# facebookresearch/dietgpu

Measured on AMD Instinct MI355X. Metric: rans_encode_decode_GBps, higher is better.
Workload: dtype u8 (byte-wise rANS on the split exponent plane of 16-bit words); 1 GPU; 256x524288 bfloat16 N(0,1), float codec, probBits 10 (BASELINE config 3); per_gpu_batch_bytes=268435456, api=C ABI: dgpu_float_compress + dgpu_float_decompress

## Files before the change

dietgpu_amd/csrc/kernels_decode.h:

```cpp
#pragma once
#include <type_traits>

#include "format.h"
#include "plan_constants.h"
#include "kernels_stats.h"

namespace dgpu {

__device__ __forceinline__ const uint8_t* locateAns(const uint8_t* archive, uint32_t ft, uint32_t* floatSize) {
  if (!ft) return archive;
  const FloatHeader fh = *(const FloatHeader*)archive;
  if (floatSize) *floatSize = fh.size;
  return archive + 16u + floatUncompDataSize(ft, fh.size);
}

struct DecodeArgs {
  BatchView in;
  BatchView out;
  uint32_t floatType;
  uint8_t* outSuccess;
  uint32_t* outSize;
  const uint32_t* inBytes;
  uint32_t numInBatch;
  uint32_t maxTiles;
// ... 128 lines not shown
  __device__ __forceinline__ void init(uint8_t* outBase, const uint8_t* archive, uint32_t, size_t first, uint32_t hl) {
    out = (uint16_t*)outBase + first + hl;
    nc = archive + 16u + first + hl;
  }
  typedef uint32_t Pre;
  typedef uint2 GroupPre;
  __device__ __forceinline__ uint32_t prefetch(uint32_t row) const { return nc[row * 32u]; }
  static __device__ __forceinline__ uint32_t joinWord(uint32_t e0, uint32_t r) {
    const uint32_t lo = joinBytes(e0, r);
    return __builtin_amdgcn_alignbit(r, lo, 1);
  }
  __device__ __forceinline__ void store(uint32_t row, uint32_t e0, uint32_t r) const {
    const uint32_t v = joinWord(e0, r);
    streamStore<kNtDecStores>(&out[row * 32u], (uint16_t)(v >> 16));
  }
  static constexpr uint32_t kXposeBytes = 512;
  __device__ __forceinline__ uint2 prefetchGroup(uint32_t g, uint32_t hl) const { return decLoad8(nc - hl + g * 256u + hl * 8u); }
  __device__ __forceinline__ void stageRow(uint32_t xpose, uint32_t j, uint32_t hl, uint32_t e0) const {
    *(LdsU16w*)(uintptr_t)(xpose + (j * 32u + hl) * 2u) = (uint16_t)(e0 >> 16);
  }
  static __device__ __forceinline__ uint32_t rotrHalves(uint32_t x) {
    typedef uint16_t u16x2w __attribute__((ext_vector_type(2)));
    const u16x2w h = __builtin_bit_cast(u16x2w, x);
    const uint32_t shifted = __builtin_bit_cast(uint32_t, (u16x2w)(h >> 1));
    uint32_t r;
    asm("v_pk_mad_u16 %0, %1, %2, %3" : "=v"(r) : "v"(x), "s"(0x80008000u), "v"(shifted));
    return r;
  }
  static __device__ __forceinline__ u32x4w joinGroup(uint32_t xpose, uint32_t hl, uint2 ncb) {
    const u32x4w v = *(const LdsU4w*)(uintptr_t)(xpose + hl * 16u);
    u32x4w o;
    o.x = rotrHalves(__builtin_amdgcn_perm(v.x, ncb.x, 0x07010500u));
    o.y = rotrHalves(__builtin_amdgcn_perm(v.y, ncb.x, 0x07030502u));
    o.z = rotrHalves(__builtin_amdgcn_perm(v.z, ncb.y, 0x07010500u));
    o.w = rotrHalves(__builtin_amdgcn_perm(v.w, ncb.y, 0x07030502u));
    return o;
  }
  __device__ __forceinline__ void flushGroup(uint32_t xpose, uint32_t g, uint32_t hl, uint2 ncb) const {
    const u32x4w o = joinGroup(xpose, hl, ncb);
    u32x4w* dst = (u32x4w*)(out - hl + g * 256u + hl * 8u);
    if (kNtDecStores) __builtin_nontemporal_store(o, dst);
    else *dst = o;
  }
};

template <>
struct RowSink<kFloat32> {
  uint32_t* out;
  const uint16_t* nc2;
  const uint8_t* nc1;
  __device__ __forceinline__ void init(uint8_t* outBase, const uint8_t* archive, uint32_t floatSize, size_t first, uint32_t hl) {
    out = (uint32_t*)outBase + first + hl;
    nc2 = (const uint16_t*)(archive + 16u) + first + hl;
    nc1 = archive + 16u + 2u * (size_t)roundUp(floatSize, 8u) + first + hl;
  }
  typedef uint32_t Pre;
  typedef uint2 GroupPre;
  __device__ __forceinline__ uint32_t prefetch(uint32_t row) const {
    return ((uint32_t)nc1[row * 32u] << 16) | nc2[row * 32u];
  }
  __device__ __forceinline__ void store(uint32_t row, uint32_t e0, uint32_t r) const {
    const uint32_t v = (e0 & 0xff000000u) | r;
    streamStore<kNtDecStores>(&out[row * 32u], (uint32_t)__builtin_amdgcn_alignbit(v, v, 1));
  }
  static __device__ __forceinline__ uint32_t joinWord(uint32_t e0, uint32_t r) {
    const uint32_t v = (e0 & 0xff000000u) | r;
    return (uint32_t)__builtin_amdgcn_alignbit(v, v, 1);
  }
  static constexpr uint32_t kXposeBytes = 0;
  __device__ __forceinline__ uint2 prefetchGroup(uint32_t, uint32_t) const { return make_uint2(0, 0); }
  __device__ __forceinline__ void stageRow(uint32_t, uint32_t, uint32_t, uint32_t) const {}
  __device__ __forceinline__ void flushGroup(uint32_t, uint32_t, uint32_t, uint2) const {}
};

template <uint32_t FT>
__device__ __forceinline__ float accWiden16(uint32_t h);
template <>
__device__ __forceinline__ float accWiden16<kFloat16>(uint32_t h) { return (float)__builtin_bit_cast(_Float16, (uint16_t)h); }
template <>
__device__ __forceinline__ float accWiden16<kBFloat16>(uint32_t h) { return __builtin_bit_cast(float, h << 16); }
__device__ __forceinline__ uint32_t accAdd(uint32_t acc, float v) { return __builtin_bit_cast(uint32_t, __fadd_rn(__builtin_bit_cast(float, acc), v)); }
typedef u32x4w u32x4w4 __attribute__((aligned(4)));

struct AccumPre {
  uint32_t r, acc;
  __device__ __forceinline__ AccumPre() = default;
  __device__ __forceinline__ AccumPre(uint32_t) : r(0), acc(0) {}
};
struct AccumGroupPre {
  uint2 nc;
  u32x4w a0, a1;
};

constexpr uint32_t kStatsSlotsLarge = 16, kStatsSlotsSmall = 8;
__host__ __device__ constexpr uint32_t decStatsSlots(uint32_t tileBlocks) { return tileBlocks <= 4u ? kStatsSlotsSmall : kStatsSlotsLarge; }
__host__ __device__ constexpr uint32_t decStatsBinBytes(uint32_t tileBlocks) { return kNumSymbols * decStatsSlots(tileBlocks) * 4u; }
typedef __attribute__((address_space(3))) uint32_t LdsU32w;
template <bool kStats>
struct AccumBins {};
template <>
struct AccumBins<true> {
  uint32_t bins;
};

template <bool kInRegisters>
struct AccumScale {};
template <>
struct AccumScale<true> {
  float scale;
  uint32_t scaleLast;
};
typedef __attribute__((address_space(3))) float LdsF32w;
__device__ __forceinline__ uint32_t accScale(uint32_t o, float f) { return __builtin_bit_cast(uint32_t, __fmul_rn(__builtin_bit_cast(float, o), f)); }

template <uint32_t FT, uint32_t kSlots = 0, bool kScaledSink = false>
struct AccumSink : AccumBins<kSlots != 0u>, AccumScale<kScaledSink && kSlots == 0u> {
  static_assert(FT == kFloat16 || FT == kBFloat16, "");
  static constexpr bool kStats = kSlots != 0u;
  static constexpr bool kScaled = kScaledSink;
  static constexpr uint32_t kStatSlots = kSlots;
  __device__ __forceinline__ bool scales() const {
    if constexpr (kStats) return this->bins != 0u;
    else return this->scaleLast != 0u;
  }
  __device__ __forceinline__ float factor() const {
    if constexpr (kStats) return *(LdsF32w*)(uintptr_t)(this->bins + kNumSymbols * kSlots * 4u);
    else return this->scale;
  }
  float* out;
  const uint8_t* nc;
  uint32_t accumulate;
  __device__ __forceinline__ void count(uint32_t o) const {
    if constexpr (kStats) {
      const uint32_t c = (castRound<FT>(o) >> (FT == kFloat16 ? 8u : 7u)) & 0xffu;
      __hip_atomic_fetch_add((LdsU32w*)(uintptr_t)(this->bins + c * (kSlots * 4u)), 1u, __ATOMIC_RELAXED, __HIP_MEMORY_SCOPE_WORKGROUP);
    }
  }
  __device__ __forceinline__ void init(uint8_t* outBase, const uint8_t* archive, uint32_t, size_t first, uint32_t hl) {
    out = (float*)outBase + first + hl;
    nc = archive + 16u + first + hl;
  }
  typedef AccumPre Pre;
  typedef AccumGroupPre GroupPre;
  __device__ __forceinline__ AccumPre prefetchAcc(uint32_t row) const {
    AccumPre p(0);
    if (accumulate) p.acc = *(const uint32_t*)&out[row * 32u];
    return p;
  }
  __device__ __forceinline__ AccumPre prefetch(uint32_t row) const {
    AccumPre p(0);
    p.r = nc[row * 32u];
    if (accumulate) p.acc = *(const uint32_t*)&out[row * 32u];
    return p;
  }
  __device__ __forceinline__ void storeWord(uint32_t row, uint32_t h, const AccumPre& p) const {
    const float v = accWiden16<FT>(h);
    uint32_t o = accumulate ? accAdd(p.acc, v) : __builtin_bit_cast(uint32_t, v);
    if constexpr (kScaled) {
      if (scales()) o = accScale(o, factor());
    }
    streamStore<kNtDecStores>((uint32_t*)&out[row * 32u], o);
    if constexpr (kStats) {
      if (this->bins) count(o);
    }
  }
  __device__ __forceinline__ void store(uint32_t row, uint32_t e0, const AccumPre& p) const {
    storeWord(row, RowSink<FT>::joinWord(e0, p.r) >> 16, p);
  }
  static constexpr uint32_t kXposeBytes = 512;
  __device__ __forceinline__ void prefetchGroupAcc(uint32_t g, uint32_t hl, AccumGroupPre& p) const {
    p.a0 = p.a1 = u32x4w{0u, 0u, 0u, 0u};
    if (accumulate) {
      const u32x4w4* src = (const u32x4w4*)(out - hl + g * 256u + hl * 8u);
      p.a0 = src[0];
      p.a1 = src[1];
    }
  }
  __device__ __forceinline__ AccumGroupPre prefetchGroup(uint32_t g, uint32_t hl) const {
    AccumGroupPre p;
    p.nc = decLoad8(nc - hl + g * 256u + hl * 8u);
    prefetchGroupAcc(g, hl, p);
    return p;
  }
  __device__ __forceinline__ void stageRow(uint32_t xpose, uint32_t j, uint32_t hl, uint32_t e0) const {
    *(LdsU16w*)(uintptr_t)(xpose + (j * 32u + hl) * 2u) = (uint16_t)(e0 >> 16);
  }
  __device__ __forceinline__ void flushGroup(uint32_t xpose, uint32_t g, uint32_t hl, const AccumGroupPre& p) const {
    flushFrom<false>(xpose, g, hl, p, u32x4w{0u, 0u, 0u, 0u});
  }
  __device__ __forceinline__ void flushWords(uint32_t g, uint32_t hl, const u32x4w& given, const AccumGroupPre& p) const {
    flushFrom<true>(0u, g, hl, p, given);
  }
  template <bool kGiven>
  __device__ __forceinline__ void flushFrom(uint32_t xpose, uint32_t g, uint32_t hl, const AccumGroupPre& p, const u32x4w& given) const {
    u32x4w w;
    if constexpr (kGiven) w = given;
    else w = RowSink<FT>::joinGroup(xpose, hl, p.nc);
    float v[8];
#pragma unroll
    for (uint32_t k = 0; k < 4u; ++k) {
      v[2u * k] = accWiden16<FT>(w[k] & 0xffffu);
      v[2u * k + 1u] = accWiden16<FT>(w[k] >> 16);
    }
    u32x4w o0, o1;
#pragma unroll
    for (uint32_t k = 0; k < 4u; ++k) {
      o0[k] = accumulate ? accAdd(p.a0[k], v[k]) : __builtin_bit_cast(uint32_t, v[k]);
      o1[k] = accumulate ? accAdd(p.a1[k], v[4u + k]) : __builtin_bit_cast(uint32_t, v[4u + k]);
    }
    if constexpr (kScaled) {
      if (scales()) {
        const float f = factor();
#pragma unroll
        for (uint32_t k = 0; k < 4u; ++k) {
          o0[k] = accScale(o0[k], f);
          o1[k] = accScale(o1[k], f);
        }
      }
    }
    u32x4w4* dst = (u32x4w4*)(out - hl + g * 256u + hl * 8u);
    if (kNtDecStores) {
      __builtin_nontemporal_store(o0, &dst[0]);
      __builtin_nontemporal_store(o1, &dst[1]);
    } else {
      dst[0] = o0;
      dst[1] = o1;
    }
    if constexpr (kStats) {
      if (this->bins) {
#pragma unroll
        for (uint32_t k = 0; k < 4u; ++k) {
          count(o0[k]);
          count(o1[k]);
        }
      }
    }
  }
};

template <uint32_t kSlots, bool kScaledSink>
struct AccumSink<kFloat32, kSlots, kScaledSink> : AccumScale<kScaledSink> {
  static_assert(kSlots == 0u, "counting sinks: the 16-bit archive types only");
  static constexpr bool kStats = false;
  static constexpr bool kScaled = kScaledSink;
  float* out;
  const uint16_t* nc2;
  const uint8_t* nc1;
  uint32_t accumulate;
  __device__ __forceinline__ void init(uint8_t* outBase, const uint8_t* archive, uint32_t floatSize, size_t first, uint32_t hl) {
    out = (float*)outBase + first + hl;
    nc2 = (const uint16_t*)(archive + 16u) + first + hl;
    nc1 = archive + 16u + 2u * (size_t)roundUp(floatSize, 8u) + first + hl;
  }
  typedef AccumPre Pre;
  typedef uint2 GroupPre;
  __device__ __forceinline__ AccumPre prefetch(uint32_t row) const {
    AccumPre p(0);
    p.r = ((uint32_t)nc1[row * 32u] << 16) | nc2[row * 32u];
    if (accumulate) p.acc = *(const uint32_t*)&out[row * 32u];
    return p;
  }
  __device__ __forceinline__ AccumPre prefetchAcc(uint32_t row) const {
    AccumPre p(0);
    if (accumulate) p.acc = *(const uint32_t*)&out[row * 32u];
    return p;
  }
  __device__ __forceinline__ void storeWord(uint32_t row, uint32_t w, const AccumPre& p) const {
    uint32_t o = accumulate ? accAdd(p.acc, __builtin_bit_cast(float, w)) : w;
    if constexpr (kScaled) {
      if (this->scaleLast != 0u) o = accScale(o, this->scale);
    }
    streamStore<kNtDecStores>((uint32_t*)&out[row * 32u], o);
  }
  __device__ __forceinline__ void store(uint32_t row, uint32_t e0, const AccumPre& p) const {
    storeWord(row, RowSink<kFloat32>::joinWord(e0, p.r), p);
  }
  static constexpr uint32_t kXposeBytes = 0;
  __device__ __forceinline__ uint2 prefetchGroup(uint32_t, uint32_t) const { return make_uint2(0, 0); }
  __device__ __forceinline__ void stageRow(uint32_t, uint32_t, uint32_t, uint32_t) const {}
  __device__ __forceinline__ void flushGroup(uint32_t, uint32_t, uint32_t, uint2) const {}
};

typedef __attribute__((address_space(3))) uint16_t LdsU16;
typedef uint32_t u32x4 __attribute__((ext_vector_type(4)));
typedef __attribute__((address_space(3))) u32x4 LdsU4;
constexpr uint32_t kRingChunkWords = 256;
constexpr uint32_t kRingBytes = 2048;
constexpr uint32_t kGroupRows = 8;

__host__ __device__ constexpr uint32_t decThreads(uint32_t tileBlocks) { return tileBlocks * 32u < 64u ? 64u : tileBlocks * 32u; }
__host__ __device__ constexpr uint32_t decXposeBytes(int P, uint32_t ft, uint32_t tileBlocks) {
  (void)P;
  if (ft == 0 && tileBlocks >= 16u) return 0u;
  return ft == kFloat32 ? 0u : 512u;
}
__host__ __device__ constexpr bool decCompactLut(int P, uint32_t tileBlocks) { return tileBlocks <= 4u || P >= 11; }
__host__ __device__ constexpr uint32_t decLutBytes(int P, uint32_t tileBlocks) {
  return decCompactLut(P, tileBlocks) ? (4u << P) : (8u << P);
}
__host__ __device__ constexpr uint32_t decLdsBytes(int P, uint32_t ft, uint32_t tileBlocks) {
  return decLutBytes(P, tileBlocks) + tileBlocks * kRingBytes + tileBlocks * decXposeBytes(P, ft, tileBlocks);
}

template <typename GroupPre>
struct DecodePreOf {
  uint4 words[4];
  GroupPre nc[2];
};
typedef DecodePreOf<uint2> DecodePre;
template <uint32_t FT, typename Sink>
__device__ __forceinline__ void decodePrefetch(DecodePreOf<typename Sink::GroupPre>& pre, const uint8_t* __restrict__ gwords, uint32_t numWords,
                                               const Sink& sink, uint32_t hl, bool wide) {
  const uint32_t paddedBytes = roundUp(numWords, kBlockAlignWords) * 2u;
#pragma unroll
  for (uint32_t k = 0; k < 4u; ++k) {
    const uint32_t off = (k * 32u + hl) * 16u;
    pre.words[k] = make_uint4(0, 0, 0, 0);
    if (off < paddedBytes) pre.words[k] = decLoad16(gwords + off);
  }
  pre.nc[0] = pre.nc[1] = typename Sink::GroupPre();
  if (wide) {
    pre.nc[0] = sink.prefetchGroup(kRowsPerBlock / 8u - 1u, hl);
    pre.nc[1] = sink.prefetchGroup(kRowsPerBlock / 8u - 2u, hl);
  }
}

template <int P, uint32_t FT, bool kFull, bool kWide = false, bool kIdleUpper = false, bool kCompact = false, bool kNoRing = false,
          bool kPre = false, bool kTail = false, typename Sink = RowSink<FT>>
__device__ __forceinline__ void decodeBlock(
    uint32_t xpose,
    uint32_t state,
    uint32_t n,
    uint32_t groups,
    const uint8_t* __restrict__ gwords,
    uint32_t numWords,
    uint32_t ringBase,
    const void* __restrict__ lutRaw,
    const Sink& sink,
    uint32_t hl,
    bool upper,
    const DecodePreOf<typename Sink::GroupPre>* pre = nullptr,
    uint32_t topRows = 0) {
  static_assert(!kPre || (kNoRing && kFull), "");
  static_assert(!kTail || (kFull && !kPre), "");
  constexpr uint32_t kMask = (1u << P) - 1u;
  const uint32_t laneMaskLt = (1u << hl) - 1u;
  auto lutAt = [&](uint32_t x) -> uint2 {
    if (kCompact) {
      const uint32_t e = ((const uint32_t*)lutRaw)[x];
      return make_uint2((e & 0xff000fffu), (e >> 12) & 0xfffu);
    }
    return ((const uint2*)lutRaw)[x];
  };
  const uint32_t paddedBytes = roundUp(numWords, kBlockAlignWords) * 2u;

  uint32_t posw = numWords;

  static_assert(!kNoRing || kFull, "whole-block staging is a full-block path");
  int lowChunk = numWords ? (int)((numWords - 1u) / kRingChunkWords) + 1 : 0;
  if (kNoRing) {
    uint4 v[4];
#pragma unroll
    for (uint32_t k = 0; k < 4u; ++k) {
      const uint32_t off = (k * 32u + hl) * 16u;
      if (kPre) {
        v[k] = pre->words[k];
      } else {
        v[k] = make_uint4(0, 0, 0, 0);
        if (off < paddedBytes) v[k] = decLoad16(gwords + off);
      }
    }
#pragma unroll
    for (uint32_t k = 0; k < 4u; ++k) {
      const uint32_t off = (k * 32u + hl) * 16u;
      if (off < paddedBytes) *(LdsU4*)(uintptr_t)(ringBase + off) = u32x4{v[k].x, v[k].y, v[k].z, v[k].w};
    }
    lowChunk = 0;
  } else {
    const int stop = numWords > 512u ? (int)((numWords - 512u) / kRingChunkWords) : 0;
    while (lowChunk > stop) {
      --lowChunk;
      const uint32_t off = (uint32_t)lowChunk * 512u + hl * 16u;
      uint4 v = make_uint4(0, 0, 0, 0);
      if (off < paddedBytes) v = decLoad16(gwords + off);
      *(LdsU4*)(uintptr_t)(ringBase | (((uint32_t)lowChunk & 3u) * 512u + hl * 16u)) = u32x4{v.x, v.y, v.z, v.w};
    }
  }
  uint4 pending = make_uint4(0, 0, 0, 0);
  int pendingChunk = -1;

  auto step = [&](bool valid) -> uint32_t {
    const uint2 e = lutAt(state & kMask);
    if (valid) state = __umul24(e.x, state >> P) + e.y;
    const bool read = valid && (state < kMinState);
    const uint64_t vote = __ballot(read);
    const uint32_t vh = upper ? (uint32_t)(vote >> 32) : (uint32_t)vote;
    posw -= __popc(vh);
    if (read) {
      const uint32_t idx = posw + __popc(vh & laneMaskLt);
      const uint32_t w = *(const LdsU16*)(uintptr_t)(((idx << 1) & (kRingBytes - 1u)) | ringBase);
      state = (state << kEncodedBits) | w;
    }
    return e.x;
  };

  typedef typename Sink::Pre Pre;
  typedef typename Sink::GroupPre GroupPre;
  uint32_t sLo = 0, sHi = 0;
  int upperSel = (upper && !kIdleUpper) ? 1 : 0;
  asm volatile("" : "+v"(upperSel));
  auto stepFull = [&]() -> uint32_t {
    const uint2 e = lutAt(state & kMask);
    state = __umul24(e.x, state >> P) + e.y;
    const bool read = state < kMinState;
    const uint64_t vote = __ballot(read);
    const uint32_t vLo = (uint32_t)vote, vHi = (uint32_t)(vote >> 32);
    const uint32_t sLoOld = sLo;
    sLo -= (uint32_t)__popc(vLo);
    sHi -= (uint32_t)__popc(vHi);
    uint32_t t = __builtin_amdgcn_mbcnt_hi(vHi, __builtin_amdgcn_mbcnt_lo(vLo, 0u));
    t = (uint32_t)(__mul24(upperSel, (int)(sHi - sLoOld)) + (int)t);
    asm volatile("" : "+v"(t));
    const uint32_t addr = kNoRing ? ((t + sLo) << 1) : ((((t + sLo) << 1) & (kRingBytes - 1u)) | ringBase);
    const uint32_t w = *(const LdsU16*)(uintptr_t)addr;
    state = read ? ((state << kEncodedBits) | w) : state;
    return e.x;
  };

  auto runGroups = [&](auto fullTag, const int gHi, const int gLo) {
    constexpr bool F = decltype(fullTag)::value;
    constexpr bool kJoinAtFlush = F && kWide;
    Pre preCur[kGroupRows], preNext[kGroupRows];
    GroupPre ncCur = GroupPre(), ncNext = GroupPre(), ncNext2 = GroupPre();
    if (kJoinAtFlush) {
      if (kPre) {
        ncCur = pre->nc[0];
        ncNext = pre->nc[1];
      } else {
        ncCur = sink.prefetchGroup((uint32_t)gHi, hl);
        ncNext = sink.prefetchGroup(gHi > gLo ? (uint32_t)(gHi - 1) : (uint32_t)gLo, hl);
      }
    }
#pragma unroll
    for (int j = 0; j < (int)kGroupRows; ++j) {
      const uint32_t row = (uint32_t)gHi * kGroupRows + j;
      preCur[j] = kJoinAtFlush ? (Pre)0 : ((F || row * 32u + hl < n) ? sink.prefetch(row) : (Pre)0);
    }

#pragma unroll 1
    for (int g = gHi; g >= gLo; --g) {
      const uint32_t gNext = g > gLo ? (uint32_t)(g - 1) : (uint32_t)gLo;
      if (kJoinAtFlush) {
        ncNext2 = sink.prefetchGroup(g > gLo + 1 ? (uint32_t)(g - 2) : (uint32_t)gLo, hl);
      } else {
#pragma unroll
        for (int j = 0; j < (int)kGroupRows; ++j) {
          const uint32_t row = gNext * kGroupRows + j;
          preNext[j] = (F || row * 32u + hl < n) ? sink.prefetch(row) : (Pre)0;
        }
      }
      if (F && !kNoRing) posw = upper ? sHi : sLo;
      if (!kNoRing) {
        if (pendingChunk >= 0) {
          *(LdsU4*)(uintptr_t)(ringBase | (((uint32_t)pendingChunk & 3u) * 512u + hl * 16u)) = u32x4{pending.x, pending.y, pending.z, pending.w};
          pendingChunk = -1;
        }
        if (lowChunk > 0 && (uint32_t)lowChunk * kRingChunkWords + 512u > posw) {
          --lowChunk;
          const uint32_t off = (uint32_t)lowChunk * 512u + hl * 16u;
          pending = (off < paddedBytes) ? decLoad16(gwords + off) : make_uint4(0, 0, 0, 0);
          pendingChunk = lowChunk;
        }
      }
#pragma unroll
      for (int j = (int)kGroupRows - 1; j >= 0; --j) {
        const uint32_t row = (uint32_t)g * kGroupRows + j;
        if (F) {
          const uint32_t e0 = stepFull();
          if (kWide) {
            if (!kIdleUpper || !upper) sink.stageRow(xpose, (uint32_t)j, hl, e0);
          } else if (!kIdleUpper || !upper) {
            sink.store(row, e0, preCur[j]);
          }
        } else {
          const bool valid = row * 32u + hl < n;
          const uint32_t e0 = step(valid);
          if (valid) sink.store(row, e0, preCur[j]);
        }
      }
      if (kJoinAtFlush) {
        if (!kIdleUpper || !upper) sink.flushGroup(xpose, (uint32_t)g, hl, ncCur);
        ncCur = ncNext;
        ncNext = ncNext2;
      } else {
#pragma unroll
        for (int j = 0; j < (int)kGroupRows; ++j) preCur[j] = preNext[j];
      }
    }
  };

  if (kTail) {
    if (topRows != 0u) runGroups(std::false_type{}, (int)(groups + divUp(topRows, kGroupRows)) - 1, (int)groups);
    if (groups == 0u) return;
  }
  if (kFull) {
    sLo = __builtin_amdgcn_readlane(posw, 0);
    sHi = __builtin_amdgcn_readlane(posw, 32);
    if (kNoRing) {
      sLo += __builtin_amdgcn_readlane(ringBase, 0) >> 1;
      sHi += __builtin_amdgcn_readlane(ringBase, 32) >> 1;
    }
  }
  runGroups(std::integral_constant<bool, kFull>{}, (int)groups - 1, 0);
}

enum class DecodeForm { kWhole, kRanged, kAccum, kReduce, kReduceStats, kReduceMixed, kReduceMixedStats, kReduceScaled, kReduceScaledStats };
template <int P, uint32_t FT, uint32_t kTileBlocks, DecodeForm kForm>
__device__ __forceinline__ void decodeTile(const DecodeArgs& a) {
  constexpr bool kRanged = kForm == DecodeForm::kRanged, kAccum = kForm == DecodeForm::kAccum;
  static_assert(kForm == DecodeForm::kWhole || kForm == DecodeForm::kRanged || kForm == DecodeForm::kAccum, "decode-reduce has a body of its own: decodeReduceTile");
  static_assert(!kAccum || FT != 0u, "accumulating decode: float archives only");
  using Sink = std::conditional_t<kAccum, AccumSink<FT ? FT : kFloat32>, RowSink<FT>>;
  constexpr uint32_t kDecThreads = decThreads(kTileBlocks);
  static_assert(kTileBlocks * kRingBytes >= 2048u, "");
  extern __shared__ __attribute__((aligned(16))) uint8_t smem[];
  uint2* sLut = (uint2*)(smem + kTileBlocks * kRingBytes);
  constexpr uint32_t kXpose = decXposeBytes(P, FT, kTileBlocks);

  const uint32_t tid = threadIdx.x;
  const uint32_t lane = tid & 63u;
  const uint32_t wave = tid >> 6;
  const bool upper = lane >= 32u;
  const uint32_t hl = lane & 31u;
  const uint32_t hw = wave * 2u + (upper ? 1u : 0u);
  uint32_t b, tile;
  if (!decodeTileOf(a, blockIdx.x, &b, &tile)) return;
  uint32_t rFirst = 0;
  uint64_t rEnd = 0;
  if constexpr (kRanged) {
    if (blockIdx.x == 0) {
      for (uint32_t e = tid; e < a.numInBatch; e += kDecThreads) {
        if (a.numBlocks[e] == 0u) {
          if (a.outSuccess) a.outSuccess[e] = 1;
          if (a.outSize) a.outSize[e] = 0;
        }
      }
    }
    if (b >= a.numInBatch) return;
    rFirst = a.firstBlock[b];
    rEnd = (uint64_t)rFirst + a.numBlocks[b];
  }
  auto rangeWords = [&](uint32_t total) -> uint32_t {
    const uint64_t lo = (uint64_t)rFirst * kBlockSize, hi = rEnd * kBlockSize;
    return lo > total ? 0u : (uint32_t)((hi < total ? hi : (uint64_t)total) - lo);
  };

  const uint8_t* archive = a.in.ptr(b);
  uint32_t floatSize = 0;
  const uint64_t inBytes = decodeInBytes(a, b);
  if (inBytes < (FT ? sizeof(FloatHeader) : sizeof(AnsHeader))) {
    if (tile == 0 && tid == 0) {
      if (a.outSuccess) a.outSuccess[b] = 0;
      if (a.outSize) a.outSize[b] = 0;
    }
    return;
  }
  if (FT) {
    const FloatHeader fh = *(const FloatHeader*)archive;
    const bool fhOk = fh.magicAndVersion == ((kFloatMagic << 16) | kFloatVersion) && (fh.options & 0xfu) == FT &&
        (kRanged || fh.size <= a.out.size(b)) &&
        (uint64_t)sizeof(FloatHeader) + floatUncompDataSize(FT, fh.size) + sizeof(AnsHeader) <= inBytes;
    if (!fhOk) {
      if (tile == 0 && tid == 0) {
        if (a.outSuccess) a.outSuccess[b] = 0;
        if (a.outSize) a.outSize[b] = kRanged ? rangeWords(fh.size) : fh.size;
      }
      return;
    }
  }
  const uint8_t* ans = locateAns(archive, FT, &floatSize);
  uint32_t block = tile * kTileBlocks + hw;
  bool inRange = true;
  if constexpr (kRanged) {
    const uint64_t blk = (uint64_t)rFirst + block;
    inRange = blk < rEnd;
    block = inRange ? (uint32_t)blk : 0u;
  }
  const bool extentKnown = inBytes != ~0ull;
  const uint32_t ansOff = ansOffsetInArchive(FT, floatSize);
  const uint32_t nbSpec = FT ? divUp(floatSize, kBlockSize) : 0u;
  const bool pdfEarly = extentKnown ? (uint64_t)ansOff + ansOverhead(0u) <= inBytes : FT != 0u;
  const bool blockEarly = FT != 0u && inRange && block < nbSpec && (!extentKnown || (uint64_t)ansOff + ansOverhead(nbSpec) <= inBytes);
  const AnsHeader header = *(const AnsHeader*)ans;
  uint2 pdfRaw = make_uint2(0u, 0u);
  if (wave == 0) pdfRaw = *(const uint2*)(pdfEarly ? ans + sizeof(AnsHeader) + 8u * lane : ans);
  uint2 bwMine = *(const uint2*)(blockEarly ? ans + ansBlockWordsOffset(nbSpec) + 8u * block : ans);
  uint32_t state = *(const uint32_t*)(blockEarly ? ans + ansStatesOffset() + 4u * (block * 32u + hl) : ans);
  const uint32_t nb = header.numBlocks;
  const uint32_t total = header.totalUncompressedWords;
  const uint32_t totalWords = header.totalCompressedWords;

  bool success = a.out.size(b) >= total;
  if constexpr (kRanged) success = (uint64_t)rFirst * kBlockSize <= total && rangeWords(total) <= a.out.size(b);
  success = success && header.magicAndVersion == ((kAnsMagic << 16) | kAnsVersion) &&
      (header.options & 0xfu) == (uint32_t)P;
  if (FT) success = success && floatSize == total;
  success = success && nb == divUp(total, kBlockSize);
  success = success && (uint64_t)ansOffsetInArchive(FT, total) + ansOverhead(nb) + 2ull * totalWords <= inBytes;
  if (!success) {
    if (tile == 0 && tid == 0) {
      if (a.outSuccess) a.outSuccess[b] = 0;
      if (a.outSize) a.outSize[b] = kRanged ? rangeWords(total) : total;
    }
    return;
  }
  uint32_t endBlock = nb, tileFirst = tile * kTileBlocks;
  if constexpr (kRanged) {
    endBlock = rEnd < nb ? (uint32_t)rEnd : nb;
    tileFirst += rFirst;
  }
  if (tileFirst >= endBlock && tile != 0) return;

  const uint2* blockWords = (const uint2*)(ans + ansBlockWordsOffset(nb));
  auto blockOk = [&](uint32_t i, uint2 bw) -> bool {
    const uint32_t want = (i + 1u < nb) ? kBlockSize : total - i * kBlockSize;
    const uint32_t words = bw.x & 0xffffu;
    return (bw.x >> 16) == want && (bw.y & (kBlockAlignWords - 1u)) == 0u &&
        (uint64_t)bw.y + roundUp(words, kBlockAlignWords) <= (uint64_t)totalWords;
  };
  bool allBlocksOk = true;
  if constexpr (kAccum) {
    for (uint32_t i = tid; i < endBlock; i += kDecThreads) allBlocksOk = blockOk(i, blockWords[i]) & allBlocksOk;
  } else if (tile == 0) {
    for (uint32_t i = rFirst + tid; i < endBlock; i += kDecThreads) allBlocksOk = allBlocksOk && blockOk(i, blockWords[i]);
  }

  bool haveBlock = inRange && block < endBlock;
  if (!haveBlock) {
    bwMine = make_uint2(0u, 0u);
    state = 0;
  } else if (!blockEarly) {
    bwMine = blockWords[block];
    state = ((const uint32_t*)(ans + ansStatesOffset()))[block * 32u + hl];
  }
  if (wave == 0 && !pdfEarly) pdfRaw = ((const uint2*)(ans + sizeof(AnsHeader)))[lane];
  uint32_t n = 0, numWords = 0, start = 0;
  if (haveBlock) {
    if (blockOk(block, bwMine)) {
      n = bwMine.x >> 16;
      numWords = bwMine.x & 0xffffu;
      start = bwMine.y;
    } else {
      haveBlock = false;
      state = 0;
    }
  }
  const uint8_t* gwords = ans + ansOverhead(nb) + 2u * (size_t)start;
  Sink sink;
  if constexpr (kAccum) sink.accumulate = a.accumulate;
  uint32_t sinkBlock = haveBlock ? block : (block & ~1u);
  if constexpr (kRanged) sinkBlock = haveBlock ? block : tileFirst + (hw & ~1u);
  sink.init(a.out.ptr(b), archive, floatSize, (size_t)sinkBlock * kBlockSize, hl);
  if constexpr (kRanged) sink.out -= (size_t)rFirst * kBlockSize;
  const uint32_t ldsBase = (uint32_t)(uintptr_t)(__attribute__((address_space(3))) uint8_t*)smem;
  const uint32_t nFirst = __shfl(n, 0, 64);
  const uint32_t nSecond = __shfl(n, 32, 64);
  const uint32_t wFirst = __shfl(numWords, 0, 64);
  const uint32_t wSecond = __shfl(numWords, 32, 64);
  const bool noRing = wFirst <= kRingBytes / 2u && wSecond <= kRingBytes / 2u;
  const bool wide = decXposeBytes(P, FT, kTileBlocks) != 0 && (kAccum || (((uintptr_t)a.out.ptr(b)) & (decOutWordBytes(FT) - 1u)) == 0);
  const bool fullPair = nFirst == kBlockSize && nSecond == kBlockSize;
  const bool fullSingle = nFirst == kBlockSize && nSecond == 0u;
  DecodePreOf<typename Sink::GroupPre> pre;
  if ((fullPair || fullSingle) && noRing) decodePrefetch<FT>(pre, gwords, numWords, sink, hl, wide);

  uint32_t* sCdf = (uint32_t*)smem;
  uint32_t* sPdf = sCdf + kNumSymbols;
  uint32_t* sPdfSum = sPdf + kNumSymbols;
  uint32_t* sWaveBad = sPdfSum + 1;
  constexpr bool kScanLut = kTileBlocks <= kDecBlocksPerSmallTile;
  uint32_t* sWaveTop = sWaveBad + 8;
  constexpr bool kCompact = decCompactLut(P, kTileBlocks);
  constexpr uint32_t kLutBytes = decLutBytes(P, kTileBlocks);
  uint8_t* sMark = (uint8_t*)sLut + kLutBytes - (1u << P);
  {
    {
      const bool waveBad = __ballot(!allBlocksOk) != 0ull;
      if (lane == 0u) sWaveBad[wave] = waveBad ? 1u : 0u;
    }
    if (kScanLut) {
      for (uint32_t i = tid; i < (1u << P) / 4u; i += kDecThreads) ((uint32_t*)sMark)[i] = 0u;
    }
    if (wave == 0) {
      const uint2 raw = pdfRaw;
      const uint32_t p0 = raw.x & 0xffffu, p1 = raw.x >> 16, p2 = raw.y & 0xffffu, p3 = raw.y >> 16;
      const uint32_t mine = p0 + p1 + p2 + p3;
      const uint32_t incl = waveInclusiveScan(mine, lane);
      const uint32_t base = incl - mine;
      ((uint4*)sCdf)[lane] = make_uint4(base, base + p0, base + p0 + p1, base + p0 + p1 + p2);
      ((uint4*)sPdf)[lane] = make_uint4(p0, p1, p2, p3);
      if (lane == 63u) *sPdfSum = incl;
    }
    __syncthreads();
    uint32_t anyBad = 0;
#pragma unroll
    for (uint32_t w = 0; w < kDecThreads / 64u; ++w) anyBad |= sWaveBad[w];
    const bool blocksOk = anyBad == 0u;
    const bool pdfOk = nb == 0u || *sPdfSum == (1u << P);
    if (tile == 0 && tid == 0) {
      if (a.outSuccess) a.outSuccess[b] = (blocksOk && pdfOk) ? 1 : 0;
      if (a.outSize) a.outSize[b] = kRanged ? rangeWords(total) : total;
    }
    if (!pdfOk || tileFirst >= endBlock) return;
    if constexpr (kAccum) {
      if (!blocksOk) return;
    }
    if constexpr (kScanLut) {
      for (uint32_t sidx = tid; sidx < kNumSymbols; sidx += kDecThreads) {
        if (sPdf[sidx]) sMark[sCdf[sidx]] = (uint8_t)sidx;
      }
      __syncthreads();
      static_assert(kCompact, "the scan build writes compact entries");
      constexpr uint32_t kWaves = kDecThreads / 64u;
      constexpr uint32_t kPart = (1u << P) / kWaves;
      static_assert(kPart % 256u == 0u, "");
      constexpr uint32_t kSteps = kPart / 256u;
      auto dmax = [](uint32_t v, uint32_t o) { return v > o ? v : o; };
      auto waveMaxScan = [&](uint32_t v) -> uint32_t {
        v = dmax(v, (uint32_t)__builtin_amdgcn_update_dpp(0, (int)v, 0x111, 0xf, 0xf, true));
        v = dmax(v, (uint32_t)__builtin_amdgcn_update_dpp(0, (int)v, 0x112, 0xf, 0xf, true));
        v = dmax(v, (uint32_t)__builtin_amdgcn_update_dpp(0, (int)v, 0x114, 0xf, 0xf, true));
        v = dmax(v, (uint32_t)__builtin_amdgcn_update_dpp(0, (int)v, 0x118, 0xf, 0xf, true));
        v = dmax(v, (uint32_t)__builtin_amdgcn_update_dpp(0, (int)v, 0x142, 0xa, 0xf, true));
        v = dmax(v, (uint32_t)__builtin_amdgcn_update_dpp(0, (int)v, 0x143, 0xc, 0xf, true));
        return v;
      };
      uint32_t m4[kSteps];
      uint32_t top = 0;
#pragma unroll
      for (uint32_t t = 0; t < kSteps; ++t) {
        m4[t] = ((const uint32_t*)sMark)[(wave * kPart + t * 256u) / 4u + lane];
        const uint32_t a01 = dmax(m4[t] & 0xffu, (m4[t] >> 8) & 0xffu);
        const uint32_t a23 = dmax((m4[t] >> 16) & 0xffu, m4[t] >> 24);
        top = dmax(top, dmax(a01, a23));
      }
      top = waveMaxScan(top);
      if (lane == 63u) sWaveTop[wave] = top;
      __syncthreads();
      uint32_t carry = 0;
      for (uint32_t w = 0; w < wave; ++w) carry = dmax(carry, sWaveTop[w]);
#pragma unroll
      for (uint32_t t = 0; t < kSteps; ++t) {
        uint32_t run[4];
        run[0] = m4[t] & 0xffu;
        run[1] = dmax(run[0], (m4[t] >> 8) & 0xffu);
        run[2] = dmax(run[1], (m4[t] >> 16) & 0xffu);
        run[3] = dmax(run[2], m4[t] >> 24);
        const uint32_t incl = waveMaxScan(run[3]);
        uint32_t excl = (uint32_t)__builtin_amdgcn_update_dpp(0, (int)incl, 0x138, 0xf, 0xf, true);
        excl = dmax(excl, carry);
        uint32_t e[4];
#pragma unroll
        for (uint32_t j = 0; j < 4u; ++j) {
          const uint32_t x = wave * kPart + t * 256u + lane * 4u + j;
          const uint32_t sym = dmax(run[j], excl);
          e[j] = (sPdf[sym] & 0xfffu) | (((x - sCdf[sym]) & 0xfffu) << 12) | (sym << 24);
        }
        ((uint4*)sLut)[(wave * kPart + t * 256u) / 4u + lane] = make_uint4(e[0], e[1], e[2], e[3]);
        carry = dmax(carry, (uint32_t)__builtin_amdgcn_readlane((int)incl, 63));
      }
    } else
    for (uint32_t x = tid; x < (1u << P); x += kDecThreads) {
      uint32_t lo = 0, hi = kNumSymbols;
#pragma unroll
      for (int it = 0; it < 8; ++it) {
        const uint32_t mid = (lo + hi) >> 1;
        const bool le = sCdf[mid] <= x;
        lo = le ? mid : lo;
        hi = le ? hi : mid;
      }
      if (kCompact) ((uint32_t*)sLut)[x] = (sPdf[lo] & 0xfffu) | (((x - sCdf[lo]) & 0xfffu) << 12) | (lo << 24);
      else sLut[x] = make_uint2((sPdf[lo] & 0xfffu) | (lo << 24), (x - sCdf[lo]) & 0xfffu);
    }
  }

  __syncthreads();

  constexpr uint32_t kLutBytesHere = decLutBytes(P, kTileBlocks);
  const uint32_t xpose = ldsBase + kTileBlocks * kRingBytes + kLutBytesHere + hw * kXpose;
  const uint32_t ringLds = ldsBase + hw * kRingBytes;
#define DGPU_DECODE_FULL(WIDE, IDLE, NORING) \
  decodeBlock<P, FT, true, WIDE, IDLE, kCompact, NORING, NORING>(xpose, state, n, kRowsPerBlock / kGroupRows, gwords, numWords, ringLds, sLut, sink, hl, upper, &pre)
  if (fullPair) {
    if (wide) {
      if (noRing) DGPU_DECODE_FULL(true, false, true); else DGPU_DECODE_FULL(true, false, false);
    } else {
      if (noRing) DGPU_DECODE_FULL(false, false, true); else DGPU_DECODE_FULL(false, false, false);
    }
  } else if (fullSingle) {
    if (wide) {
      if (noRing) DGPU_DECODE_FULL(true, true, true); else DGPU_DECODE_FULL(true, true, false);
    } else {
      if (noRing) DGPU_DECODE_FULL(false, true, true); else DGPU_DECODE_FULL(false, true, false);
    }
#undef DGPU_DECODE_FULL
  } else {
    const uint32_t maxN = nFirst > nSecond ? nFirst : nSecond;
    const uint32_t maxRows = divUp(maxN, 32u);
    const uint32_t fullRows = (nSecond ? nSecond : nFirst) / 32u;
    const uint32_t groups = fullRows / kGroupRows;
    const uint32_t topRows = maxRows - groups * kGroupRows;
    const bool tailPair = nFirst == kBlockSize && nSecond != 0u, tailSingle = nFirst != 0u && nSecond == 0u;
    if ((tailPair || tailSingle) && groups != 0u) {
#define DGPU_DECODE_TAIL(WIDE, IDLE, NORING) \
  decodeBlock<P, FT, true, WIDE, IDLE, kCompact, NORING, false, true>(xpose, state, n, groups, gwords, numWords, ringLds, sLut, sink, hl, upper, nullptr, topRows)
      if (tailPair) {
        if (wide) {
          if (noRing) DGPU_DECODE_TAIL(true, false, true); else DGPU_DECODE_TAIL(true, false, false);
        } else {
          if (noRing) DGPU_DECODE_TAIL(false, false, true); else DGPU_DECODE_TAIL(false, false, false);
        }
      } else {
        if (wide) {
          if (noRing) DGPU_DECODE_TAIL(true, true, true); else DGPU_DECODE_TAIL(true, true, false);
        } else {
          if (noRing) DGPU_DECODE_TAIL(false, true, true); else DGPU_DECODE_TAIL(false, true, false);
        }
      }
#undef DGPU_DECODE_TAIL
    } else {
      decodeBlock<P, FT, false, false, false, kCompact>(xpose, state, n, divUp(maxRows, kGroupRows), gwords, numWords, ringLds, sLut, sink, hl, upper);
    }
  }
}

constexpr uintptr_t kReduceRawTag = 1u;
__device__ __forceinline__ bool reduceIsRaw(const uint8_t* source) { return ((uintptr_t)source & kReduceRawTag) != 0u; }
typedef uint16_t u16n __attribute__((aligned(2)));
__device__ __forceinline__ uint32_t rawLoad16(const uint8_t* p) {
  return kNtEncLoads ? (uint32_t)__builtin_nontemporal_load((const u16n*)p) : (uint32_t)*(const u16n*)p;
}
__device__ __forceinline__ uint32_t rawLoad32(const uint8_t* p) {
  return kNtEncLoads ? __builtin_nontemporal_load((const uint32_t*)p) : *(const uint32_t*)p;
}
__device__ __forceinline__ u32x4w rawLoadGroup(const uint8_t* p, uint32_t align) {
  u32x4w w;
  if (align >= 16u) {
    w = kNtEncLoads ? __builtin_nontemporal_load((const u32x4w*)p) : *(const u32x4w*)p;
  } else if (align >= 4u) {
#pragma unroll
    for (uint32_t k = 0; k < 4u; ++k) w[k] = rawLoad32(p + 4u * k);
  } else {
#pragma unroll
    for (uint32_t k = 0; k < 4u; ++k) w[k] = rawLoad16(p + 4u * k) | (rawLoad16(p + 4u * k + 2u) << 16);
  }
  return w;
}
template <uint32_t FT, typename Sink>
__device__ __forceinline__ void reduceRawBlock(const Sink& sink, const uint8_t* src, uint32_t n, uint32_t hl, uint32_t align) {
  if constexpr (FT == kFloat32) {
    const uint32_t rows = n / 32u;
    uint32_t row = 0;
    for (; row + 8u <= rows; row += 8u) {
      typename Sink::Pre p[8];
      uint32_t w[8];
#pragma unroll
      for (uint32_t j = 0; j < 8u; ++j) {
        p[j] = sink.prefetchAcc(row + j);
        w[j] = rawLoad32(src + ((size_t)(row + j) * 32u + hl) * 4u);
      }
#pragma unroll
      for (uint32_t j = 0; j < 8u; ++j) sink.storeWord(row + j, w[j], p[j]);
    }
    for (; row * 32u + hl < n; ++row) {
      const typename Sink::Pre p = sink.prefetchAcc(row);
      sink.storeWord(row, rawLoad32(src + ((size_t)row * 32u + hl) * 4u), p);
    }
  } else {
    const uint32_t groups = n / (kGroupRows * 32u);
    uint32_t g = 0;
    for (; g + 4u <= groups; g += 4u) {
      typename Sink::GroupPre p[4];
      u32x4w w[4];
#pragma unroll
      for (uint32_t j = 0; j < 4u; ++j) {
        sink.prefetchGroupAcc(g + j, hl, p[j]);
        w[j] = rawLoadGroup(src + (g + j) * 512u + hl * 16u, align);
      }
#pragma unroll
      for (uint32_t j = 0; j < 4u; ++j) sink.flushWords(g + j, hl, w[j], p[j]);
    }
    for (; g < groups; ++g) {
      typename Sink::GroupPre p;
      sink.prefetchGroupAcc(g, hl, p);
      sink.flushWords(g, hl, rawLoadGroup(src + g * 512u + hl * 16u, align), p);
    }
    for (uint32_t row = groups * kGroupRows; row * 32u + hl < n; ++row) {
      const typename Sink::Pre p = sink.prefetchAcc(row);
      sink.storeWord(row, rawLoad16(src + (row * 32u + hl) * 2u), p);
    }
  }
}

__device__ __forceinline__ void reduceHandOver() {
  __builtin_amdgcn_fence(__ATOMIC_RELEASE, "workgroup");
  asm volatile("s_waitcnt vmcnt(0)" ::: "memory");
  __builtin_amdgcn_s_barrier();
  __builtin_amdgcn_fence(__ATOMIC_ACQUIRE, "workgroup");
}

__device__ __forceinline__ uint32_t reduceAccumulates(const DecodeArgs& a, uint32_t s) { return (s != 0u || a.accumulate != 0u) ? 1u : 0u; }
__device__ __forceinline__ bool reduceCounts(uint32_t s, uint32_t S) { return s + 1u == S; }
template <typename Sink>
__device__ __forceinline__ void reduceScales(Sink& sink, const DecodeArgs& a, uint32_t s) {
  if constexpr (Sink::kScaled && !Sink::kStats) {
    sink.scale = a.scale;
    sink.scaleLast = reduceCounts(s, a.numSources) ? 1u : 0u;
  }
}

template <uint32_t FT, typename Sink>
__device__ __forceinline__ void reduceRawSource(const DecodeArgs& a, uint32_t b, const uint8_t* row, uint32_t s, uint32_t total, uint32_t tileFirst,
                                                uint32_t nb, uint32_t wave, uint32_t binsLds) {
  uint32_t tidS = threadIdx.x;
  asm volatile("" : "+v"(tidS));
  const uint32_t laneS = tidS & 63u;
  const uint32_t hl = laneS & 31u;
  const uint32_t block = tileFirst + wave * 2u + (laneS >= 32u ? 1u : 0u);
  const bool haveBlock = block < nb;
  if (s != 0u) reduceHandOver();
  Sink sink;
  sink.accumulate = reduceAccumulates(a, s);
  if constexpr (Sink::kStats) sink.bins = reduceCounts(s, a.numSources) ? binsLds + (laneS & (Sink::kStatSlots - 1u)) * 4u : 0u;
  reduceScales(sink, a, s);
  sink.init(a.out.ptr(b), row, total, (size_t)(haveBlock ? block : 0u) * kBlockSize, hl);
  const uint32_t left = haveBlock ? total - block * kBlockSize : 0u;
  const uint32_t align = ((uintptr_t)row & 15u) == 0u ? 16u : (((uintptr_t)row & 3u) == 0u ? 4u : 2u);
  reduceRawBlock<FT>(sink, row + (size_t)block * kBlockSize * decOutWordBytes(FT), left < kBlockSize ? left : kBlockSize, hl, align);
}

struct ReduceSource {
  uint32_t ok;
  uint32_t total;
  uint32_t totalWords;
  uint32_t report;
};
constexpr uint32_t kMaxReduceSources = 64;

template <int P, uint32_t FT, uint32_t kTileBlocks, bool kStats = false, bool kMixed = false, bool kScaled = false>
__device__ __forceinline__ void decodeReduceTile(const DecodeArgs& a) {
  static_assert(FT != 0u, "decode-reduce: float archives only");
  constexpr uint32_t kSlots = kStats ? decStatsSlots(kTileBlocks) : 0u;
  using Sink = AccumSink<FT, kSlots, kScaled>;
  constexpr uint32_t kDecThreads = decThreads(kTileBlocks), kWaves = kDecThreads / 64u;
  extern __shared__ __attribute__((aligned(16))) uint8_t smem[];
  uint2* sLut = (uint2*)(smem + kTileBlocks * kRingBytes);
  constexpr uint32_t kXpose = decXposeBytes(P, FT, kTileBlocks);
  static_assert(kTileBlocks * kRingBytes >= 4096u + kMaxReduceSources * sizeof(ReduceSource) + 4u * kWaves, "");
  ReduceSource* sSrc = (ReduceSource*)(smem + 4096u);
  uint32_t* sWaveBad = (uint32_t*)(sSrc + kMaxReduceSources);

  const uint32_t tid = threadIdx.x;
  const uint32_t lane = tid & 63u;
  const uint32_t wave = (uint32_t)__builtin_amdgcn_readfirstlane((int)(tid >> 6));
  uint32_t b, tile;
  if (!decodeTileOf(a, blockIdx.x, &b, &tile)) return;
  const uint32_t S = a.numSources, first = b * S;
  const uint32_t capacity = a.out.size(b);
  const uint32_t tileFirst = tile * kTileBlocks;
  if (tile != 0 && (uint64_t)tileFirst * kBlockSize >= capacity) return;
  constexpr uint32_t kBinsAt = kTileBlocks * kRingBytes + decLutBytes(P, kTileBlocks) + kTileBlocks * kXpose;
  if constexpr (kStats) {
    for (uint32_t i = tid; i < kNumSymbols * kSlots / 4u; i += kDecThreads) ((uint4*)(smem + kBinsAt))[i] = make_uint4(0u, 0u, 0u, 0u);
    if constexpr (kScaled) {
      if (tid < kSlots) ((float*)(smem + kBinsAt + decStatsBinBytes(kTileBlocks)))[tid] = a.scale;
    }
  }

  for (uint32_t s = wave; s < S; s += kWaves) {
    const uint8_t* archive = a.in.ptr(first + s);
    const uint64_t inBytes = a.inBytes[first + s];
    ReduceSource r = {0u, 0u, 0u, 0u};
    bool raw = false;
    if constexpr (kMixed) raw = reduceIsRaw(archive);
    if (raw) {
      const uint32_t words = (uint32_t)(inBytes / decOutWordBytes(FT));
      r.ok = (kStats ? words == capacity : words <= capacity) ? 1u : 0u;
      r.total = r.report = words;
    } else if (inBytes >= sizeof(FloatHeader)) {
      const FloatHeader fh = *(const FloatHeader*)archive;
      r.report = fh.size;
      const bool fhOk = fh.magicAndVersion == ((kFloatMagic << 16) | kFloatVersion) && (fh.options & 0xfu) == FT && fh.size <= capacity &&
          (uint64_t)sizeof(FloatHeader) + floatUncompDataSize(FT, fh.size) + sizeof(AnsHeader) <= inBytes;
      if (fhOk) {
        const uint8_t* ans = archive + ansOffsetInArchive(FT, fh.size);
        const AnsHeader header = *(const AnsHeader*)ans;
        const uint32_t nb = header.numBlocks, total = header.totalUncompressedWords;
        bool ok = capacity >= total && header.magicAndVersion == ((kAnsMagic << 16) | kAnsVersion) && (header.options & 0xfu) == (uint32_t)P &&
            fh.size == total && nb == divUp(total, kBlockSize) &&
            (uint64_t)ansOffsetInArchive(FT, total) + ansOverhead(nb) + 2ull * header.totalCompressedWords <= inBytes;
        if constexpr (kStats) ok = ok && total == capacity;
        if (ok && nb != 0u) {
          const uint2 raw = *(const uint2*)(ans + sizeof(AnsHeader) + 8u * lane);
          uint32_t sum = (raw.x & 0xffffu) + (raw.x >> 16) + (raw.y & 0xffffu) + (raw.y >> 16);
#pragma unroll
          for (int d = 32; d >= 1; d >>= 1) sum += __shfl_xor(sum, d, 64);
          ok = sum == (1u << P);
        }
        r.ok = ok ? 1u : 0u;
        r.total = total;
        r.totalWords = header.totalCompressedWords;
        r.report = total;
      }
    }
    if (lane == 0u) sSrc[s] = r;
  }
  __syncthreads();
  const uint32_t total = sSrc[0].total, report = sSrc[0].report;
  bool memberOk = true;
  for (uint32_t s = 0; s < S; ++s) memberOk = memberOk && sSrc[s].ok != 0u && sSrc[s].total == total;
  if (!memberOk) {
    if (tile == 0 && tid == 0) {
      if (a.outSuccess) a.outSuccess[b] = 0;
      if (a.outSize) a.outSize[b] = report;
    }
    return;
  }
  const uint32_t nb = divUp(total, kBlockSize);
  if (tileFirst >= nb && tile != 0) return;
  const uint32_t ansOff = ansOffsetInArchive(FT, total);
  {
    bool allBlocksOk = true;
    for (uint32_t i = tid; i < S * nb; i += kDecThreads) {
      const uint32_t s = i / nb, blk = i - s * nb;
      if constexpr (kMixed) {
        if (reduceIsRaw(a.in.ptr(first + s))) continue;
      }
      const uint2 bw = ((const uint2*)(a.in.ptr(first + s) + ansOff + ansBlockWordsOffset(nb)))[blk];
      const uint32_t want = (blk + 1u < nb) ? kBlockSize : total - blk * kBlockSize;
      const bool ok = (bw.x >> 16) == want && (bw.y & (kBlockAlignWords - 1u)) == 0u &&
          (uint64_t)bw.y + roundUp(bw.x & 0xffffu, kBlockAlignWords) <= (uint64_t)sSrc[s].totalWords;
      allBlocksOk = allBlocksOk & ok;
    }
    const bool waveBad = __ballot(!allBlocksOk) != 0ull;
    if (lane == 0u) sWaveBad[wave] = waveBad ? 1u : 0u;
  }
  __syncthreads();
  uint32_t anyBad = 0;
#pragma unroll
  for (uint32_t w = 0; w < kWaves; ++w) anyBad |= sWaveBad[w];
  if (tile == 0 && tid == 0) {
    if (a.outSuccess) a.outSuccess[b] = anyBad ? 0 : 1;
    if (a.outSize) a.outSize[b] = report;
  }
  if (anyBad != 0u || tileFirst >= nb) return;

  const uint32_t ldsBase = (uint32_t)(uintptr_t)(__attribute__((address_space(3))) uint8_t*)smem;
  constexpr bool kCompact = decCompactLut(P, kTileBlocks);
  const bool wide = kXpose != 0u;
  uint32_t* sCdf = (uint32_t*)smem;
  uint32_t* sPdf = sCdf + kNumSymbols;

#pragma unroll 1
  for (uint32_t s = 0; s < S; ++s) {
    if constexpr (kMixed) {
      const uint8_t* src = a.in.ptr(first + s);
      if (reduceIsRaw(src)) {
        reduceRawSource<FT, Sink>(a, b, src - kReduceRawTag, s, total, tileFirst, nb, wave, ldsBase + kBinsAt);
        continue;
      }
    }
    uint32_t tidS = threadIdx.x;
    asm volatile("" : "+v"(tidS));
    const uint32_t laneS = tidS & 63u;
    const bool upper = laneS >= 32u;
    const uint32_t hl = laneS & 31u;
    const uint32_t hw = wave * 2u + (upper ? 1u : 0u);
    const uint32_t block = tileFirst + hw;
    const bool haveBlock = block < nb;
    const uint32_t sinkBlock = haveBlock ? block : (block & ~1u);
    const uint32_t xpose = ldsBase + kTileBlocks * kRingBytes + decLutBytes(P, kTileBlocks) + hw * kXpose;
    const uint32_t ringLds = ldsBase + hw * kRingBytes;
    const uint8_t* archive = a.in.ptr(first + s);
    const uint8_t* ans = archive + ansOff;
    uint2 pdfRaw = make_uint2(0u, 0u), bwMine = make_uint2(0u, 0u);
    uint32_t state = 0;
    if (wave == 0) pdfRaw = ((const uint2*)(ans + sizeof(AnsHeader)))[laneS];
    if (haveBlock) {
      bwMine = ((const uint2*)(ans + ansBlockWordsOffset(nb)))[block];
      state = ((const uint32_t*)(ans + ansStatesOffset()))[block * 32u + hl];
    }
    if (s != 0u) reduceHandOver();
    const uint32_t n = bwMine.x >> 16, numWords = bwMine.x & 0xffffu;
    const uint8_t* gwords = ans + ansOverhead(nb) + 2u * (size_t)bwMine.y;
    Sink sink;
    sink.accumulate = reduceAccumulates(a, s);
    if constexpr (kStats) sink.bins = reduceCounts(s, S) ? ldsBase + kBinsAt + (laneS & (kSlots - 1u)) * 4u : 0u;
    reduceScales(sink, a, s);
    sink.init(a.out.ptr(b), archive, total, (size_t)sinkBlock * kBlockSize, hl);
    const uint32_t nFirst = __shfl(n, 0, 64);
    const uint32_t nSecond = __shfl(n, 32, 64);
    const uint32_t wFirst = __shfl(numWords, 0, 64);
    const uint32_t wSecond = __shfl(numWords, 32, 64);
    const bool noRing = wFirst <= kRingBytes / 2u && wSecond <= kRingBytes / 2u;
    const bool fullPair = nFirst == kBlockSize && nSecond == kBlockSize;
    const bool fullSingle = nFirst == kBlockSize && nSecond == 0u;
    DecodePreOf<typename Sink::GroupPre> pre;
    if ((fullPair || fullSingle) && noRing) decodePrefetch<FT>(pre, gwords, numWords, sink, hl, wide);

    if (wave == 0) {
      const uint32_t p0 = pdfRaw.x & 0xffffu, p1 = pdfRaw.x >> 16, p2 = pdfRaw.y & 0xffffu, p3 = pdfRaw.y >> 16;
      const uint32_t mine = p0 + p1 + p2 + p3;
      const uint32_t base = waveInclusiveScan(mine, laneS) - mine;
      ((uint4*)sCdf)[laneS] = make_uint4(base, base + p0, base + p0 + p1, base + p0 + p1 + p2);
      ((uint4*)sPdf)[laneS] = make_uint4(p0, p1, p2, p3);
    }
    __syncthreads();
    for (uint32_t x = tidS; x < (1u << P); x += kDecThreads) {
// ... 124 lines not shown
```

Before: 2323 GB/s.

## Rotate group non-compressed prefetch registers in decode for 16-bit float sinks

Measured after the change: 2300 GB/s. 1.0% lower.

```diff
diff --git a/dietgpu_amd/csrc/kernels_decode.h b/dietgpu_amd/csrc/kernels_decode.h
--- a/dietgpu_amd/csrc/kernels_decode.h
+++ b/dietgpu_amd/csrc/kernels_decode.h
@@ -454,6 +454,19 @@
   return decLutBytes(P, tileBlocks) + tileBlocks * kRingBytes + tileBlocks * decXposeBytes(P, ft, tileBlocks);
 }
 
+template <typename Sink>
+struct GroupPreRenamed {
+  static constexpr int kAhead = 0;
+};
+template <>
+struct GroupPreRenamed<RowSink<kFloat16>> {
+  static constexpr int kAhead = 2;
+};
+template <>
+struct GroupPreRenamed<RowSink<kBFloat16>> {
+  static constexpr int kAhead = 2;
+};
+
 template <typename GroupPre>
 struct DecodePreOf {
   uint4 words[4];
@@ -478,7 +491,8 @@
 }
 
 template <int P, uint32_t FT, bool kFull, bool kWide = false, bool kIdleUpper = false, bool kCompact = false, bool kNoRing = false,
-          bool kPre = false, bool kTail = false, typename Sink = RowSink<FT>>
+          bool kPre = false, bool kTail = false, typename Sink = RowSink<FT>,
+          bool kRenameGroups = false>
 __device__ __forceinline__ void decodeBlock(
     uint32_t xpose,
     uint32_t state,
@@ -582,6 +596,52 @@
   auto runGroups = [&](auto fullTag, const int gHi, const int gLo) {
     constexpr bool F = decltype(fullTag)::value;
     constexpr bool kJoinAtFlush = F && kWide;
+    constexpr int kAhead = kRenameGroups ? GroupPreRenamed<Sink>::kAhead : 0;
+    if constexpr (kJoinAtFlush && kAhead != 0) {
+      GroupPre r[kAhead + 1];
+      if (kPre) {
+        r[0] = pre->nc[0];
+        r[1] = pre->nc[1];
+      } else {
+        r[0] = sink.prefetchGroup((uint32_t)gHi, hl);
+        r[1] = sink.prefetchGroup(gHi > gLo ? (uint32_t)(gHi - 1) : (uint32_t)gLo, hl);
+      }
+#pragma unroll
+      for (int i = 2; i < kAhead; ++i) r[i] = sink.prefetchGroup(gHi > gLo + i - 1 ? (uint32_t)(gHi - i) : (uint32_t)gLo, hl);
+      auto group = [&](const int g, const GroupPre& cur, GroupPre& fill) {
+        fill = sink.prefetchGroup(g > gLo + kAhead - 1 ? (uint32_t)(g - kAhead) : (uint32_t)gLo, hl);
+        if (!kNoRing) {
+          posw = upper ? sHi : sLo;
+          if (pendingChunk >= 0) {
+            *(LdsU4*)(uintptr_t)(ringBase | (((uint32_t)pendingChunk & 3u) * 512u + hl * 16u)) = u32x4{pending.x, pending.y, pending.z, pending.w};
+            pendingChunk = -1;
+          }
+          if (lowChunk > 0 && (uint32_t)lowChunk * kRingChunkWords + 512u > posw) {
+            --lowChunk;
+            const uint32_t off = (uint32_t)lowChunk * 512u + hl * 16u;
+            pending = (off < paddedBytes) ? decLoad16(gwords + off) : make_uint4(0, 0, 0, 0);
+            pendingChunk = lowChunk;
+          }
+        }
+#pragma unroll
+        for (int j = (int)kGroupRows - 1; j >= 0; --j) {
+          const uint32_t e0 = stepFull();
+          if (!kIdleUpper || !upper) sink.stageRow(xpose, (uint32_t)j, hl, e0);
+        }
+        if (!kIdleUpper || !upper) sink.flushGroup(xpose, (uint32_t)g, hl, cur);
+      };
+      int g = gHi;
+#pragma unroll 1
+      for (; g >= gLo + kAhead; g -= kAhead + 1) {
+#pragma unroll
+        for (int i = 0; i <= kAhead; ++i) group(g - i, r[i], r[(i + kAhead) % (kAhead + 1)]);
+      }
+#pragma unroll
+      for (int i = 0; i < kAhead; ++i) {
+        if (g - i >= gLo) group(g - i, r[i], r[(i + kAhead) % (kAhead + 1)]);
+      }
+      return;
+    }
     Pre preCur[kGroupRows], preNext[kGroupRows];
     GroupPre ncCur = GroupPre(), ncNext = GroupPre(), ncNext2 = GroupPre();
     if (kJoinAtFlush) {
@@ -942,7 +1002,7 @@
   const uint32_t xpose = ldsBase + kTileBlocks * kRingBytes + kLutBytesHere + hw * kXpose;
   const uint32_t ringLds = ldsBase + hw * kRingBytes;
 #define DGPU_DECODE_FULL(WIDE, IDLE, NORING) \
-  decodeBlock<P, FT, true, WIDE, IDLE, kCompact, NORING, NORING>(xpose, state, n, kRowsPerBlock / kGroupRows, gwords, numWords, ringLds, sLut, sink, hl, upper, &pre)
+  decodeBlock<P, FT, true, WIDE, IDLE, kCompact, NORING, NORING, false, Sink, true>(xpose, state, n, kRowsPerBlock / kGroupRows, gwords, numWords, ringLds, sLut, sink, hl, upper, &pre)
   if (fullPair) {
     if (wide) {
       if (noRing) DGPU_DECODE_FULL(true, false, true); else DGPU_DECODE_FULL(true, false, false);
@@ -965,7 +1025,7 @@
     const bool tailPair = nFirst == kBlockSize && nSecond != 0u, tailSingle = nFirst != 0u && nSecond == 0u;
     if ((tailPair || tailSingle) && groups != 0u) {
 #define DGPU_DECODE_TAIL(WIDE, IDLE, NORING) \
-  decodeBlock<P, FT, true, WIDE, IDLE, kCompact, NORING, false, true>(xpose, state, n, groups, gwords, numWords, ringLds, sLut, sink, hl, upper, nullptr, topRows)
+  decodeBlock<P, FT, true, WIDE, IDLE, kCompact, NORING, false, true, Sink, true>(xpose, state, n, groups, gwords, numWords, ringLds, sLut, sink, hl, upper, nullptr, topRows)
       if (tailPair) {
         if (wide) {
           if (noRing) DGPU_DECODE_TAIL(true, false, true); else DGPU_DECODE_TAIL(true, false, false);
```
